# khanhptnk/magical-1

Measured on AMD Instinct MI355X. Metric: env-steps/sec (whole node) at N instances/GPU, 1/2/4/8 MI355X, higher is better.
Workload: dtype f64

## Files before the change

### include/magical_sim.h

```cpp
#ifndef MAGICAL_SIM_H
#define MAGICAL_SIM_H
#include <stdint.h>

#ifdef __cplusplus
extern "C" {
#endif

typedef struct mg_sim mg_sim;

typedef struct {
    int32_t task;
    int32_t rand_flags;
    int32_t preproc;
    int32_t num_envs;
    int32_t device;
    int32_t max_episode_steps;
    uint32_t base_seed;
    int32_t auto_reset;
    const uint32_t *seeds;
    const void *library;
    int64_t library_size;
} mg_config;

typedef struct {
// ... 25 lines not shown
int mg_read_timing(mg_sim *sim, double *out);
int mg_set_episode_steps(mg_sim *sim, const int32_t *steps_dev, void *stream);
int mg_replay_lores(const uint8_t *frames, int32_t nframes, const int32_t *episode_start, int32_t preproc,
                    uint8_t *scratch, uint8_t *out_allo, uint8_t *out_ego, uint8_t *out_past, void *stream);
int mg_restack(const uint8_t *recv, int32_t world, int32_t n, int64_t rank_stride, int64_t off_allo, int64_t off_ego,
               int64_t off_done, int32_t preproc, int64_t step, int32_t all_fresh, uint8_t *ring, uint8_t *out_allo,
               uint8_t *out_ego, uint8_t *out_past, void *stream);
int mg_restack_window(const uint8_t *recv, int32_t world, int32_t n, int64_t rank_stride, int64_t off_allo,
                      int64_t off_ego, int64_t off_done, int32_t preproc, int64_t step, int32_t all_fresh, int32_t K,
                      uint8_t *ring, void *stream);
int mg_bind_window(mg_sim *sim, uint8_t *ring_allo, uint8_t *ring_ego, int32_t K);
int mg_window_start(const mg_sim *sim, int32_t *slot);
int64_t mg_snapshot_bytes(const mg_config *cfg, int32_t n);
int mg_snapshot(mg_sim *sim, const int32_t *envs, int32_t n, uint8_t *blob_dev, void *stream);
int mg_restore(mg_sim *sim, const uint8_t *blob_dev, const int32_t *envs, const int32_t *recs, int32_t n, void *stream);
typedef struct {
    double  *score;
    int32_t *steps;
    double  *bodies;
    int32_t *counts;
    int32_t *errors;
} mg_lookahead_out;
int mg_lookahead(mg_sim *sim, const uint8_t *actions_dev, int32_t H, const mg_lookahead_out *out, void *stream);
#define MG_PLAN_MAX_ROLLOUTS 262144
typedef struct {
    int32_t *best;
    double  *best_score;
    uint8_t *first_action;
    double  *scores;
    int32_t *steps;
// ... 59 lines not shown
```

### magical-1_amd/csrc/mg_pool.h

```cpp
#pragma once
#include <hip/hip_runtime.h>
#include <functional>
#include <vector>
#include "mg_state.h"

enum { ROW_STATE = 0, ROW_RNG = 1 };
struct StateRow { uint64_t off; uint32_t esize, kind; };

__device__ __forceinline__ void copy_elem(char *dst, const char *src, uint32_t esize) {
    switch (esize) {
    case 8: *(uint64_t *)dst = *(const uint64_t *)src; break;
    case 4: *(uint32_t *)dst = *(const uint32_t *)src; break;
    case 2: *(uint16_t *)dst = *(const uint16_t *)src; break;
    default: *dst = *src; break;
    }
}

struct Carver {
    char *base;
    size_t off;
    std::vector<StateRow> *rows = nullptr;
    size_t N = 0;
    uint32_t kind = ROW_STATE;
    template <typename T> T *take(size_t n) {
        off = (off + 255) & ~(size_t)255;
        T *p = (T *)(base ? base + off : nullptr);
        if (rows)
            for (size_t k = 0; k < n / N; k++) rows->push_back(StateRow{off + k * N * sizeof(T), (uint32_t)sizeof(T), kind});
        off += n * sizeof(T);
        return p;
    }
};

inline void layout(MGState &S, Carver &c, bool frames = true) {
    size_t N = (size_t)S.N;
    c.N = N;
    size_t B = MG_MAX_BODIES * N, SH = MG_MAX_SHAPES * N, C = MG_MAX_CONS * N, A = MG_MAX_ARB * N, E = MG_MAX_ENTS * N;
    S.bpx = c.take<double>(B); S.bpy = c.take<double>(B); S.bvx = c.take<double>(B); S.bvy = c.take<double>(B);
    S.ba = c.take<double>(B); S.bw = c.take<double>(B); S.bvbx = c.take<double>(B); S.bvby = c.take<double>(B);
    S.bwb = c.take<double>(B); S.brc = c.take<double>(B); S.brs = c.take<double>(B); S.bminv = c.take<double>(B);
    S.biinv = c.take<double>(B); S.bacache = c.take<double>(B); S.bkin = c.take<int8_t>(B);
    S.nbodies = c.take<int32_t>(N);
    S.sbody = c.take<int8_t>(SH); S.spoly = c.take<int8_t>(SH); S.sent = c.take<int8_t>(SH);
    S.sgroup = c.take<int16_t>(SH); S.shash = c.take<int16_t>(SH); S.scat = c.take<uint8_t>(SH);
    S.sr = c.take<double>(SH); S.su = c.take<double>(SH); S.sbbl = c.take<double>(SH); S.sbbb = c.take<double>(SH);
    S.sbbr = c.take<double>(SH); S.sbbt = c.take<double>(SH);
    S.nshapes = c.take<int32_t>(N);
    S.ctype = c.take<int8_t>(C); S.ca = c.take<int8_t>(C); S.cb = c.take<int8_t>(C);
    S.cp = c.take<double>((size_t)CP_NUM * C);
// ... 13 lines not shown
    S.target_speed = c.take<double>(N); S.rel_turn = c.take<double>(N); S.target_finger = c.take<double>(N);
    S.robot_body0 = c.take<int32_t>(N); S.robot_cons0 = c.take<int32_t>(N); S.pv = c.take<double>(5 * N);
    S.ekind = c.take<int8_t>(E); S.etype = c.take<int8_t>(E); S.ecol = c.take<int8_t>(E); S.erole = c.take<int8_t>(E);
    S.ebody0 = c.take<int8_t>(E); S.eshape0 = c.take<int8_t>(E); S.enshapes = c.take<int8_t>(E);
    S.ex = c.take<double>(E); S.ey = c.take<double>(E); S.eang = c.take<double>(E); S.eh = c.take<double>(E);
    S.ew = c.take<double>(E); S.nents = c.take<int32_t>(N);
    S.goal_ent = c.take<int32_t>(N); S.episode_steps = c.take<int32_t>(N);
    S.tgt_ent = c.take<int32_t>(N); S.tgt_ids = c.take<int32_t>(2 * N);
    S.tgt_x = c.take<double>(N); S.tgt_y = c.take<double>(N);
    S.target_out = nullptr;
    c.kind = ROW_RNG;
    S.mt_key = c.take<uint32_t>(624 * N);
    c.kind = ROW_STATE;
    S.mt_pos = c.take<int32_t>(N);
    c.rows = nullptr;
    if (!frames) { S.hist_allo = S.hist_ego = S.scache = S.scache_ok = nullptr; S.hist_head = nullptr; return; }
    size_t FR = (size_t)MG_LORES * MG_LORES * 3;
    S.hist_allo = c.take<uint8_t>(4 * N * FR); S.hist_ego = c.take<uint8_t>(4 * N * FR);
    S.hist_head = c.take<int32_t>(2 * N);
    S.scache = c.take<uint8_t>(N * FR); S.scache_ok = c.take<uint8_t>(N);
}

struct StatePool { MGState S = {}; void *mem = nullptr; size_t bytes = 0; std::vector<StateRow> rows; };

inline void pool_free(StatePool &p) {
    (void)hipFree(p.mem);
    p = StatePool();
}

inline hipError_t pool_create(StatePool &p, const MGState &proto, int N, bool frames,
                              const std::function<void(Carver &)> &extra = nullptr) {
    p.S = proto;
    p.S.N = N;
    Carver sizing = {nullptr, 0};
    layout(p.S, sizing, frames);
    if (extra) extra(sizing);
    p.bytes = sizing.off + 256;
    hipError_t err = hipMalloc(&p.mem, p.bytes);
    if (err == hipSuccess) err = hipMemset(p.mem, 0, p.bytes);
    if (err != hipSuccess) { pool_free(p); return err; }
    Carver real = {(char *)p.mem, 0};
    real.rows = &p.rows;
    layout(p.S, real, frames);
    if (extra) extra(real);
    return hipSuccess;
// ... 10 lines not shown
```

### magical-1_amd/csrc/mg_render.h

```cpp
#pragma once
#include "mg_launch.h"
#include "mg_step.h"
#include "mg_prof.h"
#include <type_traits>

#define RG_LARGE 160, 1600, 256, 3072, 1600, MG_MAX_ENTS, uint32_t
#ifndef RG_MEDIUM0
#define RG_MEDIUM0 44, 784, 128, 1280, 512, MG_MAX_ENTS, uint16_t
#endif
#ifndef RG_MEDIUM1
#define RG_MEDIUM1 48, 896, 160, 1536, 512, MG_MAX_ENTS, uint16_t
#endif
#ifndef RG_MEDIUM2
#define RG_MEDIUM2 96, 1280, 160, 2560, 768, MG_MAX_ENTS, uint16_t, 16
#endif
#ifndef RG_SMALL
#define RG_SMALL 28, 640, 160, 1536, 208, 4, uint8_t, 16, 4
#endif
#define RG_MAXLONG 16
#define RG_MAXDE 16
#define RG_THREADS 192
#ifndef RG_SHORT
#define RG_SHORT 12
#endif
// ... 372 lines not shown
        } else if (x == MG_XF_PUPIL_L || x == MG_XF_PUPIL_R) {
            mg_transform_tr(0.0, 0.0, AT(S.ba, b + 2 + (x - MG_XF_PUPIL_L)) - AT(S.ba, b), xf);
        }
    } else if (kind == MG_ENT_BLOCK && x == MG_XF_MAIN) {
        const int b = AT(S.ebody0, ent);
        body_sincos(S, e, b, s, c);
        mg_transform_tr_sc(AT(S.bpx, b), AT(S.bpy, b), s, c, xf);
    } else if (kind == MG_ENT_GOAL && x == MG_XF_MAIN) {
        mg_transform_tr(AT(S.ex, ent), AT(S.ey, ent), 0.0, xf);
    }
}

template <class SM>
MG_DEV int xf_slot(int ent, int x) { return x == MG_XF_MAIN ? ent : SM::RG_MAXE + x - 1; }

#ifndef RG_SMALL_WPE
#define RG_SMALL_WPE 7
#endif
template <class SM, int MODE>
__global__ void __launch_bounds__(RG_THREADS)
__attribute__((amdgpu_waves_per_eu((SM::RG_MAXG <= 32 && RG_SMALL_WPE) ? RG_SMALL_WPE : 1)))
render_kernel(MGState S, const mg_library *__restrict__ L, RenderOut out) {
    __shared__ SM sm;
    constexpr int RG_BAND = SM::BAND, RG_NBANDS = SM::NBANDS, RG_BROWS = SM::BROWS;
    constexpr int RG_STKT = RG_BROWS * MG_LORES / 4, RG_RING0 = RG_STKT > 64 ? RG_STKT : 64;
    constexpr int RG_BANDLO = RG_BROWS * RG_LOROW, RG_BANDLO16 = SM::BANDLO16;
    constexpr int RG_CPF0 = RG_THREADS - RG_BANDLO16 < 128 ? RG_THREADS - RG_BANDLO16 : 128;
    constexpr int mode = MODE == 2 ? 0 : MODE;
    constexpr bool WIN = MODE == 2;
    const int e = blockIdx.x, view = blockIdx.y, tid = threadIdx.x, lane = tid & 63;
// ... 1 lines not shown
    if (out.retry_in) {
        const bool restart = out.cls_level == out.first_level && S.episode_steps[e] == 0;
        const int stored = S.rg_retry[2 * e + view];
        const int lvl = restart || stored < out.first_level ? out.first_level : stored;
        if (lvl != out.cls_level) return;
        if (tid == 0 && stored != lvl) S.rg_retry[2 * e + view] = (uint8_t)lvl;
    }
    if (mode == 0 && view == 0 && tid == 0 && S.scache_ok && S.episode_steps[e] == 0) S.scache_ok[e] = 0;
    MG_PROF_BEGIN(tid == 0);
#define RG_FAIL() do { \
        if (tid == 0) { if (out.retry_out) S.rg_retry[2 * e + view] = (uint8_t)(out.cls_level + 1); \
                        else S.overflow[e] |= 4 << view; } \
        return; } while (0)
    const int nents = S.nents[e];
    if (nents > SM::RG_MAXE || (out.retry_out && out.force_retry > out.cls_level - out.first_level)) RG_FAIL();
    int my_r0 = 0, my_nr = 0;
    if (tid < nents) {
        int kind = AT(S.ekind, tid);
        if (kind == MG_ENT_ARENA) { my_r0 = L->arena_rpoly0; my_nr = L->arena_nrpoly; }
        else if (kind == MG_ENT_GOAL) { my_r0 = L->goal_rpoly0; my_nr = L->goal_nrpoly; }
        else if (kind == MG_ENT_ROBOT) { my_r0 = L->robot_rpoly0; my_nr = L->robot_nrpoly; }
        else { int t = AT(S.etype, tid); my_r0 = L->block_rpoly0[t]; my_nr = L->block_nrpoly[t]; }
        sm.u.pre.e_g0[tid + 1] = (int16_t)my_nr;
        sm.u.pre.e_r0[tid] = (int16_t)my_r0;
        sm.u.pre.ocnt[tid] = 0;
    }
    if (tid == 0) {
        sm.err = 0; sm.ndash = 0; sm.nsedge = 0; sm.nlong = 0; sm.u.pre.ndedge = 0; sm.u.pre.nconv = 0;
        sm.col[0] = pack_rgb(L->background);
        sm.u.pre.e_g0[0] = 0;
// ... 78 lines not shown
            const int gk = goff[k];
#else
            const int gk = sm.u.pre.e_g0[k];
#endif
            if (k < nents && gk <= g) { ent = k; g0 = gk; }
        }
        const int r = sm.u.pre.e_r0[ent] + g - g0;
        const mg_rpoly &rp = L->rpoly[r];
        const int ecol = AT(S.ecol, ent);
        sm.u.pre.g_rpoly[g] = (int16_t)r;
        sm.g_ent[g] = (int8_t)ent;
        if (rp.outline) {
            if (atomicAdd(&sm.u.pre.ocnt[ent], 1) != 0) sm.err = 6;
            sm.oord1[ent + 1] = (uint16_t)((2 * g + 2) << RG_OSH);
        }
        sm.g_nv[g] = (int16_t)rp.npts;
        sm.col[2 * g + 1] = ref_colour(L, rp.col_ref, ecol);
        sm.col[2 * g + 2] = rp.outline ? ref_colour(L, rp.ocol_ref, ecol) : 0ull;
    }
    RG_SYNC();
    if (tid < 64) wave_exclusive_scan(sm.g_nv, sm.g_voff, G, lane);
    MG_PROF(11);
    for (int g = tid; g < G; g += RG_THREADS) {
        const mg_rpoly &rp = L->rpoly[sm.u.pre.g_rpoly[g]];
        int ent = sm.g_ent[g];
        double M[9];
        for (int i = 0; i < 9; i++) M[i] = sm.u.pre.view[i];
        for (int k = rp.nxf - 1; k >= 0; k--) {
            int x = rp.xf[k];
            const double *T = x >= MG_XF_STATIC0 ? L->static_xf[x - MG_XF_STATIC0] : sm.u.pre.e_xf[xf_slot<SM>(ent, x)];
            mg_mat3_mul(M, T, M);
        }
        for (int i = 0; i < 6; i++) sm.u.pre.g_m[g][i] = M[i];
    }
    RG_SYNC();
    const int NV = sm.g_voff[G];
    if (NV > SM::RG_MAXVERT) RG_FAIL();
    for (int g = tid; g < G; g += RG_THREADS)
        for (int i = 0, v0 = sm.g_voff[g]; i < sm.g_nv[g]; i++) sm.v_geom[v0 + i] = (uint8_t)g;
    RG_SYNC();
// ... 164 lines not shown
    uint8_t *ring = view == 0 ? S.hist_allo : S.hist_ego;
    const size_t FR = (size_t)MG_LORES * MG_LORES * 3;
    const bool fresh = S.episode_steps[e] == 0;
    const int head = S.hist_head[view * S.N + e];
    const int nh = fresh ? 0 : ((head + 1) & 3);
    const int pp = out.preproc;
    const bool fo = out.frames_only != 0;
    const bool stacked0 = !fo && (pp == MG_PREPROC_LORESSTACK || (pp == MG_PREPROC_LORES4E && view == 1) ||
                                  (pp == MG_PREPROC_LORES4A && view == 0));
    uint8_t *const wring = (WIN && stacked0) ? out.wring[view] : nullptr;
    const bool win = WIN && wring != nullptr;
    const bool stacked = stacked0 && !win;
    const bool plain = fo || pp != MG_PREPROC_LORESSTACK;
    const bool keep_ring = stacked || (!fo && pp == MG_PREPROC_LORES3EA && view == 1);
    constexpr bool kLayer = RG_SCACHE && SM::RG_MAXG <= 32;
    const bool cview = kLayer && mode == 0 && view == 0 && out.scache_mode != 1 && !keep_ring && !stacked0 && plain;
    const bool mk_cache = cview && fresh && !SM::ORDMAX;
    const bool use_cache = cview && !fresh && S.scache_ok[e] != 0;
    uint8_t *const scache = S.scache + (size_t)e * FR;
    uint4 cpf = make_uint4(0, 0, 0, 0);
    uint8_t *o_plain = view == 0 ? out.obs_allo : out.obs_ego;
    uint8_t *o_stack = pp == MG_PREPROC_LORESSTACK ? o_plain : out.obs_past;
    const int oyl = lane >> 5, ox = 32 * (tid >> 6) + (lane & 31), x0 = 4 * ox;
    const bool do_pf = mode == 0 && stacked && !fresh && tid < RG_STKT;
#ifdef MG_PROFILE
    const int dskip = out.debug_skip;
#else
    const int dskip = 0;
#endif
    uint32_t pf[3][3];
    auto prefetch = [&](int y0) {
#pragma unroll
        for (int k = 0; k < 3; k++) {
            const int sl = (nh + 1 + k) & 3;
// ... 234 lines not shown
                    uint32_t w0, w1;
                    if constexpr (SM::MPW == 8) { w0 = sm.u.post.band[yb + r][ox >> 1] >> (16 * (ox & 1)); w1 = 0u; }
                    else if constexpr (SM::MPW == 4) { w0 = sm.u.post.band[yb + r][ox]; w1 = 0u; }
                    else { const uint2 t = *(const uint2 *)&sm.u.post.band[yb + r][2 * ox]; w0 = t.x; w1 = t.y; }
                    if (w0 | w1) {
#pragma unroll
                        for (int c = 0; c < 4; c++) {
                            const uint32_t wc = (SM::MPW >= 4 || c < 2) ? w0 : w1;
                            const uint32_t m = (wc >> (SM::MBITS * (c % SM::MPW))) & (sonly ? sm.smask : SM::MMASK);
                            const uint32_t oo = sm.oord1[m ? 32 - __clz((int)m) : 0];
                            o[r][c] = o[r][c] > oo ? o[r][c] : oo;
                        }
                    }
                }
            }
            uint64_t sum = 0;
#pragma unroll
            for (int r = 0; r < 4; r++)
#pragma unroll
                for (int c = 0; c < 4; c++) sum += *(const uint64_t *)((const char *)sm.col + (o[r][c] << (3 - RG_OSH)));
            if (mode == 1) {
                for (int r = 0; r < 4; r++) {
                    uint8_t *dst = out.full + ((((size_t)e * 2 + view) * MG_RES + y0 + yb + r) * MG_RES + x0) * 3;
                    for (int c = 0; c < 4; c++) {
                        const uint64_t cc = *(const uint64_t *)((const char *)sm.col + (o[r][c] << (3 - RG_OSH)));
                        dst[3 * c] = (uint8_t)cc; dst[3 * c + 1] = (uint8_t)(cc >> 16); dst[3 * c + 2] = (uint8_t)(cc >> 32);
                    }
                }
            } else {
                uint8_t *dst8 = sonly ? (uint8_t *)sm.u.post.los : lo8;
// ... 75 lines not shown
                dst[0] = make_uint4(o[0], o[1], o[2], o[3]);
                dst[1] = make_uint4(o[4], o[5], o[6], o[7]);
                dst[2] = make_uint4(o[8], o[9], o[10], o[11]);
            }
        }
        if (band_i + 1 < band1) {
            if (tid >= 128) band_list(y0 + RG_BAND);
            if (do_pf) prefetch(y0 + RG_BAND);
            cache_prefetch(y0 + RG_BAND);
        }
        RG_SYNC();
        MG_PROF(4);
    }
    if (sm.err) { if (tid == 0) S.overflow[e] |= 4 << view; }
    if (mode == 0 && tid == 0) S.hist_head[view * S.N + e] = nh;
    if (cview && fresh && tid == 0) S.scache_ok[e] = mk_cache ? 1 : 0;
    MG_PROF_END(16 * view);
}
#undef RG_FAIL
```

### magical-1_amd/csrc/mg_sim.hip

```cpp
#include <cstdio>
#include <cstring>
#include <cstdlib>

#include "mg_sim.h"
#include "mg_phys.h"
#include "mg_philox.h"

static thread_local std::string g_err;
int set_err(int code, const std::string &msg) {
    g_err = msg;
    return code;
}

__global__ void __launch_bounds__(64) bodies_kernel(MGState S, double *out, int32_t *counts) {
    int e = blockIdx.x * blockDim.x + threadIdx.x;
    if (e >= S.n_envs) return;
    for (int b = 0; b < MG_MAX_BODIES; b++) {
        double *o = out + ((size_t)e * MG_MAX_BODIES + b) * 6;
        if (b < S.nbodies[e]) {
            o[0] = AT(S.bpx, b); o[1] = AT(S.bpy, b); o[2] = AT(S.ba, b);
            o[3] = AT(S.bvx, b); o[4] = AT(S.bvy, b); o[5] = AT(S.bw, b);
        } else {
            for (int k = 0; k < 6; k++) o[k] = 0.0;
        }
// ... 145 lines not shown
    s->max_steps = cfg->max_episode_steps; s->auto_reset = cfg->auto_reset;
    auto env_int = [](const char *name, int unset) { const char *v = getenv(name); return v ? atoi(v) : unset; };
    MGState proto = {};
    proto.n_envs = cfg->num_envs;
    proto.cons_cap = MG_MAX_CONS;
    proto.arb_cap = MG_MAX_ARB;
    proto.max_tries = 10000;
    if (env_int("MG_DEBUG_MAX_TRIES", 0) > 0) proto.max_tries = env_int("MG_DEBUG_MAX_TRIES", 0);
    s->reset_waves = env_int("MG_RESET_WAVES", 0);
    s->no_fused_reset = env_int("MG_FUSED_RESET", 1) == 0;
    s->reset_waves_shadow = env_int("MG_RESET_WAVES_SHADOW", 256);
    s->copy_wg = env_int("MG_COPY_WG", 2048);
    s->force_render_retry = env_int("MG_DEBUG_RENDER_RETRY", 0);
    s->scache_mode = env_int("MG_DEBUG_SCACHE", 0);
    const int N = (cfg->num_envs + 63) / 64 * 64;
    hipError_t err = pool_create(s->main, proto, N, true);
    if (err != hipSuccess) return set_err(-12, std::string("mg_create: state pool: ") + hipGetErrorString(err));
    if (hipMalloc((void **)&s->dlib, sizeof(mg_library)) != hipSuccess) return set_err(-12, "mg_create: hipMalloc library");
    HIPC(hipMemcpy(s->dlib, cfg->library, sizeof(mg_library), hipMemcpyHostToDevice));
    s->caps = step_caps(cfg->task, cfg->rand_flags, ((const mg_library *)cfg->library)->block_nshapes[MG_SHAPE_STAR]);
    s->step_form = step_pick_form(s->caps, env_int("MG_STEP_VARIANT", -1));
    int cus = 256;
    (void)hipDeviceGetAttribute(&cus, hipDeviceAttributeMultiprocessorCount, s->device);
    s->step_blk = step_pick_blk(s->step_form, cfg->num_envs, cus, env_int("MG_STEP_BLK", 0), env_int("MG_STEP_BLK0", 0));
    if (hipMalloc((void **)&s->reset_mask, (size_t)N) != hipSuccess) return set_err(-12, "mg_create: hipMalloc mask");
    HIPC(hipMemset(s->reset_mask, 0, (size_t)N));
    bool prefetch = s->auto_reset && s->task != MG_TASK_MOVE_TO_REGION && s->task != MG_TASK_MOVE_TO_CORNER;
    if (const char *pf = getenv("MG_RESET_PREFETCH")) prefetch = s->auto_reset && atoi(pf) != 0;
    if (prefetch) {
        HIPC(pool_create(s->shadow, proto, N, false));
        const std::vector<StateRow> &rows = s->main.rows;
// ... 299 lines not shown
```

### magical-1_amd/csrc/mg_snapshot.h

```cpp
#pragma once
#include <hip/hip_runtime.h>
#include <stdint.h>
#include "mg_common.h"

#define MG_SNAP_MAGIC 0x4E53474Du
#define MG_SNAP_VERSION 1
#define MG_SNAP_HEADER_BYTES 256
#define MG_SNAP_FRAME_BYTES (MG_LORES * MG_LORES * 3)
#define MG_SNAP_MAX_FRAMES 8

struct SnapHeader {
    uint32_t magic, version;
    int32_t task, rand_flags, preproc;
    int32_t max_bodies, max_shapes, max_cons, max_arb, max_ents;
    int32_t nrows, nframes;
    int64_t state_bytes, record_bytes, count, total_bytes;
    uint8_t zero[MG_SNAP_HEADER_BYTES - 12 * 4 - 4 * 8];
};
static_assert(sizeof(SnapHeader) == MG_SNAP_HEADER_BYTES, "SnapHeader is the blob's first 256 bytes");

struct SnapRow { uint64_t off; uint32_t esize, pre; };

struct SnapFrames { int n; uint8_t *base[MG_SNAP_MAX_FRAMES]; };

static inline int snap_frame_count(int preproc) {
    switch (preproc) {
    case MG_PREPROC_LORES4E: case MG_PREPROC_LORES3EA: return 6;
    case MG_PREPROC_LORESSTACK: return 8;
    case MG_PREPROC_LORES4A: return 5;
    default: return 0;
    }
}

hipError_t mg_launch_snap_header(const SnapHeader &h, uint8_t *blob, hipStream_t st);
hipError_t mg_launch_snap_state(char *pool, char *state, const SnapRow *rows, int nrows, const int32_t *envs,
                                const int32_t *recs, int n, int64_t count, int to_blob, hipStream_t st);
hipError_t mg_launch_snap_frames(const SnapFrames &F, uint8_t *frames, const int32_t *envs, const int32_t *recs, int n,
                                 int to_blob, hipStream_t st);
struct SnapRebuild { const uint8_t *ring[2]; const int32_t *head[2]; uint8_t *plain[2]; uint8_t *stack[2]; int N; };
hipError_t mg_launch_snap_rebuild(const SnapRebuild &R, const int32_t *envs, int n, hipStream_t st);
hipError_t mg_launch_snap_target(const int32_t *tgt_ids, const double *tgt_x, const double *tgt_y, int N,
                                 double *target_out, const int32_t *envs, int n, hipStream_t st);
```

### magical-1_amd/csrc/mg_snapshot.hip

```cpp
#include <cstring>

#include "mg_sim.h"

#define SNAP_MAX_WG 2048
#define SNAP_ROWS_PER_WG 8

__global__ void __launch_bounds__(64) snap_header_kernel(SnapHeader h, uint32_t *blob) {
    blob[threadIdx.x] = ((const uint32_t *)&h)[threadIdx.x];
}

template <bool TO_BLOB>
__global__ void __launch_bounds__(256) snap_state_kernel(char *__restrict__ pool, char *__restrict__ state,
                                                         const SnapRow *__restrict__ rows, int nrows,
                                                         const int32_t *__restrict__ envs, const int32_t *__restrict__ recs,
                                                         int n, int64_t count) {
    const int nrb = (n + 255) / 256, nrg = (nrows + SNAP_ROWS_PER_WG - 1) / SNAP_ROWS_PER_WG;
    for (int64_t item = blockIdx.x; item < (int64_t)nrb * nrg; item += gridDim.x) {
        const int k = (int)(item % nrb) * 256 + threadIdx.x;
        if (k >= n) continue;
        const size_t e = envs ? envs[k] : k, rec = recs ? recs[k] : k;
        const int r0 = (int)(item / nrb) * SNAP_ROWS_PER_WG, r1 = r0 + SNAP_ROWS_PER_WG < nrows ? r0 + SNAP_ROWS_PER_WG : nrows;
        for (int r = r0; r < r1; r++) {
            const SnapRow w = rows[r];
            char *p = pool + w.off + e * w.esize;
// ... 59 lines not shown
            dst[2] = make_uint4(o[8], o[9], o[10], o[11]);
        }
    }
}

__global__ void __launch_bounds__(64) snap_target_kernel(const int32_t *__restrict__ tgt_ids, const double *__restrict__ tgt_x,
                                                         const double *__restrict__ tgt_y, int N, double *__restrict__ out,
                                                         const int32_t *__restrict__ envs, int n) {
    const int k = blockIdx.x * 64 + threadIdx.x;
    if (k >= n) return;
    const size_t e = envs ? envs[k] : k;
    double *t = out + 4 * e;
    t[0] = tgt_ids[e]; t[1] = tgt_ids[N + e]; t[2] = tgt_x[e]; t[3] = tgt_y[e];
}

static unsigned capped(int64_t items) { return (unsigned)(items < SNAP_MAX_WG ? (items > 0 ? items : 1) : SNAP_MAX_WG); }

hipError_t mg_launch_snap_header(const SnapHeader &h, uint8_t *blob, hipStream_t st) {
    hipLaunchKernelGGL(snap_header_kernel, dim3(1), dim3(64), 0, st, h, (uint32_t *)blob);
    return hipGetLastError();
}

hipError_t mg_launch_snap_state(char *pool, char *state, const SnapRow *rows, int nrows, const int32_t *envs,
                                const int32_t *recs, int n, int64_t count, int to_blob, hipStream_t st) {
    if (n <= 0 || nrows <= 0) return hipSuccess;
    const int64_t items = (int64_t)((n + 255) / 256) * ((nrows + SNAP_ROWS_PER_WG - 1) / SNAP_ROWS_PER_WG);
    if (to_blob)
        hipLaunchKernelGGL(snap_state_kernel<true>, dim3(capped(items)), dim3(256), 0, st, pool, state, rows, nrows, envs,
                           recs, n, count);
    else
        hipLaunchKernelGGL(snap_state_kernel<false>, dim3(capped(items)), dim3(256), 0, st, pool, state, rows, nrows, envs,
                           recs, n, count);
    return hipGetLastError();
}

hipError_t mg_launch_snap_frames(const SnapFrames &F, uint8_t *frames, const int32_t *envs, const int32_t *recs, int n,
                                 int to_blob, hipStream_t st) {
    if (n <= 0 || F.n <= 0) return hipSuccess;
    const int64_t items = (int64_t)n * F.n;
    if (to_blob)
        hipLaunchKernelGGL(snap_frames_kernel<true>, dim3(capped(items)), dim3(192), 0, st, F, frames, envs, recs, n);
    else
        hipLaunchKernelGGL(snap_frames_kernel<false>, dim3(capped(items)), dim3(192), 0, st, F, frames, envs, recs, n);
    return hipGetLastError();
}

hipError_t mg_launch_snap_rebuild(const SnapRebuild &R, const int32_t *envs, int n, hipStream_t st) {
    if (n <= 0 || (!R.ring[0] && !R.ring[1])) return hipSuccess;
    const int64_t blocks = ((int64_t)n * (MG_LORES * MG_LORES / 4) + 255) / 256;
    hipLaunchKernelGGL(snap_rebuild_kernel, dim3(capped(blocks), 2), dim3(256), 0, st, R, envs, n);
    return hipGetLastError();
}

hipError_t mg_launch_snap_target(const int32_t *tgt_ids, const double *tgt_x, const double *tgt_y, int N,
                                 double *target_out, const int32_t *envs, int n, hipStream_t st) {
    if (n <= 0) return hipSuccess;
    hipLaunchKernelGGL(snap_target_kernel, dim3((n + 63) / 64), dim3(64), 0, st, tgt_ids, tgt_x, tgt_y, N, target_out,
                       envs, n);
// ... 99 lines not shown
        HIPC(hipEventCreateWithFlags(&s->ev_snap, hipEventDisableTiming));
    }
    if (s->snap_inflight) HIPC(hipEventSynchronize(s->ev_snap));
    s->snap_inflight = 0;
    int32_t *he = (int32_t *)s->snap_stage, *hr = he + ne;
    uint8_t *hm = (uint8_t *)(hr + ne);
    for (int k = 0; k < n; k++) { he[k] = envs ? envs[k] : k; hr[k] = recs ? recs[k] : k; }
    if (want_mask) {
        memset(hm, 0, (size_t)s->main.S.N);
        for (int k = 0; k < n; k++) hm[he[k]] = 1;
    }
    HIPC(hipMemcpyAsync(s->snap_dev, s->snap_stage, bytes, hipMemcpyHostToDevice, st));
    *envs_dev = (const int32_t *)s->snap_dev;
    *recs_dev = *envs_dev + ne;
    if (mask_dev) *mask_dev = (const uint8_t *)(*recs_dev + ne);
    return 0;
}

int mg_snapshot(mg_sim *s, const int32_t *envs, int32_t n, uint8_t *blob, void *stream) {
    if (!s || !blob) return set_err(-22, "mg_snapshot: null argument");
    if ((uintptr_t)blob & 15) return set_err(-22, "mg_snapshot: the blob must be 16-byte aligned");
    if (int rc = snap_check_mode(s, "mg_snapshot")) return rc;
    if (n <= 0 || n > s->main.S.n_envs || (!envs && n != s->main.S.n_envs))
        return set_err(-22, "mg_snapshot: n must be in [1, num_envs], and num_envs when envs is null");
    for (int k = 0; envs && k < n; k++)
        if (envs[k] < 0 || envs[k] >= s->main.S.n_envs) return set_err(-22, "mg_snapshot: env index out of range");
    HIPC(hipSetDevice(s->device));
    hipStream_t st = as_stream(stream);
    const int32_t *de = nullptr, *dr = nullptr;
    if (envs) {
// ... 45 lines not shown
        const int64_t r = recs ? recs[k] : k;
        if (r < 0 || r >= h.count) return set_err(-22, "mg_restore: record index out of range (the blob holds " +
                                                            std::to_string(h.count) + ")");
    }
    const bool all = n == ne;
    const int32_t *de = nullptr, *dr = nullptr;
    const uint8_t *dm = nullptr;
    const bool staged = envs || recs || !all;
    if (staged) {
        if (int rc = snap_stage_indices(s, st, envs, recs, n, true, &de, &dr, &dm)) return rc;
        if (all) dm = nullptr;
    }
    const char *state = (const char *)blob + MG_SNAP_HEADER_BYTES;
    HIPC(mg_launch_snap_state((char *)s->main.mem, (char *)state, s->srows, s->nsrows, de, dr, n, h.count, 0, st));
    HIPC(mg_launch_snap_frames(snap_frames(s), (uint8_t *)state + h.count * h.state_bytes, de, dr, n, 0, st));
    SnapRebuild R;
    memset(&R, 0, sizeof(R));
    R.N = s->main.S.N;
    const int pp = s->preproc;
    if (pp == MG_PREPROC_LORESSTACK || pp == MG_PREPROC_LORES4A) {
        R.ring[0] = s->main.S.hist_allo; R.head[0] = s->main.S.hist_head;
        R.plain[0] = pp == MG_PREPROC_LORES4A ? s->out.obs_allo : nullptr;
        R.stack[0] = pp == MG_PREPROC_LORES4A ? s->out.obs_past : s->out.obs_allo;
    }
    if (pp == MG_PREPROC_LORESSTACK || pp == MG_PREPROC_LORES4E || pp == MG_PREPROC_LORES3EA) {
        R.ring[1] = s->main.S.hist_ego; R.head[1] = s->main.S.hist_head + s->main.S.N;
        R.plain[1] = pp == MG_PREPROC_LORESSTACK ? nullptr : s->out.obs_ego;
        R.stack[1] = pp == MG_PREPROC_LORESSTACK ? s->out.obs_ego : pp == MG_PREPROC_LORES4E ? s->out.obs_past : nullptr;
    }
    HIPC(mg_launch_snap_rebuild(R, de, n, st));
// ... 14 lines not shown
```

### magical-1_amd/csrc/mg_state.h

```cpp
#pragma once
#include "mg_common.h"

struct MGState {
    int N;
    int n_envs;
    int cons_cap, arb_cap;
    int max_tries;
    double *bpx, *bpy, *bvx, *bvy, *ba, *bw, *bvbx, *bvby, *bwb, *brc, *brs, *bminv, *biinv, *bacache;
    int8_t *bkin;
    int32_t *nbodies;
    int8_t *sbody, *spoly, *sent;
    int16_t *sgroup, *shash;
    uint8_t *scat;
    double *sr, *su, *sbbl, *sbbb, *sbbr, *sbbt;
    int32_t *nshapes;
    int8_t *ctype, *ca, *cb;
    double *cp;
    int32_t *ncons;
    int32_t *akey;
    uint32_t *astamp;
    int8_t *astate, *acount, *asa, *asb;
    double *anx, *any, *au;
    double *acon;
    uint64_t *ahash;
// ... 10 lines not shown
    double *ex, *ey, *eang, *eh, *ew;
    int32_t *nents;
    int32_t *goal_ent;
    int32_t *episode_steps;
    int32_t *tgt_ent, *tgt_ids;
    double *tgt_x, *tgt_y;
    double *target_out;
    uint32_t *mt_key;
    int32_t *mt_pos;
    uint32_t *mt_lds;
    uint8_t *hist_allo;
    uint8_t *hist_ego;
    int32_t *hist_head;
    uint8_t *scache;
    uint8_t *scache_ok;
};

enum {
    CP_MAXF = 0, CP_MAXB = 1, CP_BCOEF = 2, CP_JACC = 3, CP_JACC2 = 4, CP_ISUM = 5, CP_BIAS = 6, CP_BIAS2 = 7,
    CP_AAX = 8, CP_AAY = 9, CP_ABX = 10, CP_ABY = 11, CP_R1X = 12, CP_R1Y = 13, CP_R2X = 14, CP_R2Y = 15,
    CP_K11 = 16, CP_K12 = 17, CP_K21 = 18, CP_K22 = 19,
    CP_PHASE = 8, CP_RATIO = 9, CP_RATIO_INV = 10,
    CP_MIN = 8, CP_MAX = 9,
    CP_RATE = 8,
    CP_REST = 8, CP_STIFF = 9, CP_WCOEF = 10, CP_TWRN = 11,
    CP_NUM = 20
};
enum { AC_R1X = 0, AC_R1Y, AC_R2X, AC_R2Y, AC_NMASS, AC_TMASS, AC_JN, AC_JT, AC_JB, AC_BIAS, AC_NUM };
enum { ARB_FIRST = 0, ARB_NORMAL = 1, ARB_CACHED = 3 };
```

### magical-1_amd/magical_amd/envs.py

```python
import collections
import ctypes

import numpy as np
import torch

from . import native, registry, spaces, tables
from .planning import as_objective

_LIBRARY = None


def library():
    global _LIBRARY
    if _LIBRARY is None:
        _LIBRARY = tables.build_library()
    return _LIBRARY


def _obs_shapes(spec):
    pp = spec.preproc
    if pp is None:
        return collections.OrderedDict([("allo", (384, 384, 3)), ("ego", (384, 384, 3))])
    if pp == "LoResStack":
        return collections.OrderedDict([("allo", (96, 96, 12)), ("ego", (96, 96, 12))])
# ... 233 lines not shown
        out = (ctypes.c_int32 * 6)()
        native.check(self.lib.mg_step_form(self.handle, out))
        return int(out[0]), int(out[1]), tuple(int(x) for x in out[2:6])

    def arbiters(self):
        out = torch.empty((self.num_envs, 48, 28), dtype=torch.float64, device=self.device)
        hs = torch.empty((self.num_envs, 48, 2), dtype=torch.uint64, device=self.device)
        native.check(self.lib.mg_get_arbiters(self.handle, ctypes.c_void_p(out.data_ptr()),
                                              ctypes.c_void_p(hs.data_ptr()), self._stream()))
        return out, hs

    def set_body_pose(self, env, body, x, y, angle):
        native.check(self.lib.mg_set_body_pose(self.handle, int(env), int(body), float(x), float(y), float(angle),
                                               self._stream()))

    def errors(self):
        out = torch.empty(self.num_envs, dtype=torch.int32, device=self.device)
        native.check(self.lib.mg_get_errors(self.handle, ctypes.c_void_p(out.data_ptr()), self._stream()))
        return out

    def snapshot_bytes(self, n=None):
        nbytes = self.lib.mg_snapshot_bytes(ctypes.byref(self._cfg), self.num_envs if n is None else int(n))
        if nbytes < 0:
            native.check(int(nbytes))
        return int(nbytes)

    def snapshot(self, envs=None, out=None):
        from .snapshot import Snapshot
        n = self.num_envs if envs is None else len(envs)
        nbytes = self.snapshot_bytes(n)
# ... 330 lines not shown
```

### magical-1_amd/magical_amd/native.py

```python
import ctypes
import os

HERE = os.path.dirname(os.path.abspath(__file__))
LIB_PATH = os.path.join(HERE, "libmagical_sim_prof.so" if os.environ.get("MAGICAL_AMD_PROFILE") == "1"
                        else "libmagical_sim.so")
if os.environ.get("MAGICAL_AMD_EXP_LIB"):
    LIB_PATH = os.path.join(HERE, "libmagical_sim_%s.so" % os.path.basename(os.environ["MAGICAL_AMD_EXP_LIB"]))

EXPORTS = ["mg_create", "mg_bind_outputs", "mg_reset", "mg_step", "mg_render_full", "mg_get_bodies", "mg_get_arbiters",
           "mg_set_body_pose", "mg_get_errors", "mg_seed", "mg_random_actions", "mg_num_envs", "mg_step_form", "mg_enable_timing", "mg_read_timing",
           "mg_set_episode_steps", "mg_selftest_sincos", "mg_replay_lores", "mg_restack", "mg_restack_window", "mg_bind_window",
           "mg_window_start", "mg_snapshot_bytes", "mg_snapshot", "mg_restore", "mg_lookahead", "mg_plan", "mg_plan_sample",
           "mg_plan_cem", "mg_lookahead_obj", "mg_plan_obj", "mg_plan_cem_obj", "mg_plan_beam", "mg_destroy", "mg_last_error"]
PLAN_MAX_ROLLOUTS = 262144
OBJ_FINAL, OBJ_RETURN, OBJ_PEAK = 0, 1, 2


class mg_config(ctypes.Structure):
    _fields_ = [("task", ctypes.c_int32), ("rand_flags", ctypes.c_int32), ("preproc", ctypes.c_int32),
                ("num_envs", ctypes.c_int32), ("device", ctypes.c_int32), ("max_episode_steps", ctypes.c_int32),
                ("base_seed", ctypes.c_uint32), ("auto_reset", ctypes.c_int32),
                ("seeds", ctypes.POINTER(ctypes.c_uint32)), ("library", ctypes.c_void_p),
                ("library_size", ctypes.c_int64)]


class mg_buffers(ctypes.Structure):
    _fields_ = [("obs_allo", ctypes.c_void_p), ("obs_ego", ctypes.c_void_p), ("obs_past", ctypes.c_void_p),
# ... 77 lines not shown
    if hasattr(lib, "mg_replay_lores"):
        lib.mg_replay_lores.argtypes = [vp, i32, vp, i32, vp, vp, vp, vp, vp]
    if hasattr(lib, "mg_restack"):
        i64 = ctypes.c_int64
        lib.mg_restack.argtypes = [vp, i32, i32, i64, i64, i64, i64, i32, i64, i32, vp, vp, vp, vp, vp]
    if hasattr(lib, "mg_restack_window"):
        i64 = ctypes.c_int64
        lib.mg_restack_window.argtypes = [vp, i32, i32, i64, i64, i64, i64, i32, i64, i32, i32, vp, vp]
    if hasattr(lib, "mg_bind_window"):
        lib.mg_bind_window.argtypes = [vp, vp, vp, i32]
        lib.mg_window_start.argtypes = [vp, ctypes.POINTER(i32)]
    lib.mg_snapshot_bytes.argtypes = [ctypes.POINTER(mg_config), i32]
    lib.mg_snapshot_bytes.restype = ctypes.c_int64
    lib.mg_snapshot.argtypes = [vp, ctypes.POINTER(i32), i32, vp, vp]
    lib.mg_restore.argtypes = [vp, vp, ctypes.POINTER(i32), ctypes.POINTER(i32), i32, vp]
    lib.mg_lookahead.argtypes = [vp, vp, i32, ctypes.POINTER(mg_lookahead_out), vp]
    lib.mg_plan.argtypes = [vp, vp, i32, i32, ctypes.POINTER(mg_plan_out), vp]
    lib.mg_plan_sample.argtypes = [vp, vp, i32, i32, i32, u64, u64, vp]
    lib.mg_plan_cem.argtypes = [vp, vp, vp, i32, i32, i32, i32, i32, i32, i32, u64, u64,
                                ctypes.POINTER(mg_plan_cem_out), vp]
    po = ctypes.POINTER(mg_objective)
    lib.mg_lookahead_obj.argtypes = [vp, vp, i32, po, ctypes.POINTER(mg_lookahead_out), ctypes.POINTER(mg_objective_out), vp]
    lib.mg_plan_obj.argtypes = [vp, vp, i32, i32, po, ctypes.POINTER(mg_plan_out), vp]
    lib.mg_plan_cem_obj.argtypes = [vp, vp, vp, i32, i32, i32, i32, i32, i32, i32, u64, u64, po,
                                    ctypes.POINTER(mg_plan_cem_out), vp]
    lib.mg_plan_beam.argtypes = [vp, vp, vp, i32, i32, i32, i32, po, ctypes.POINTER(mg_plan_beam_out), vp]
    lib.mg_destroy.argtypes = [vp]
    lib.mg_destroy.restype = None
    lib.mg_last_error.restype = ctypes.c_char_p
    for name in EXPORTS[:-2]:
# ... 14 lines not shown
```

Measured before the change: 3.477 million.

## Cache static-layer ordering per env to render only dynamic bodies

```diff
diff --git a/include/magical_sim.h b/include/magical_sim.h
--- a/include/magical_sim.h
+++ b/include/magical_sim.h
@@ -63,6 +63,8 @@
 int64_t mg_snapshot_bytes(const mg_config *cfg, int32_t n);
 int mg_snapshot(mg_sim *sim, const int32_t *envs, int32_t n, uint8_t *blob_dev, void *stream);
 int mg_restore(mg_sim *sim, const uint8_t *blob_dev, const int32_t *envs, const int32_t *recs, int32_t n, void *stream);
+int mg_layer_levels(mg_sim *sim, uint8_t *out_host);
+int32_t mg_restored_layer_level(int32_t stored);
 typedef struct {
     double  *score;
     int32_t *steps;
diff --git a/magical-1_amd/csrc/mg_pool.h b/magical-1_amd/csrc/mg_pool.h
--- a/magical-1_amd/csrc/mg_pool.h
+++ b/magical-1_amd/csrc/mg_pool.h
@@ -32,7 +32,8 @@
     }
 };
 
-inline void layout(MGState &S, Carver &c, bool frames = true) {
+enum { FRAMES_NONE = 0, FRAMES = 1, FRAMES_SORD = 2 };
+inline void layout(MGState &S, Carver &c, int frames = FRAMES) {
     size_t N = (size_t)S.N;
     c.N = N;
     size_t B = MG_MAX_BODIES * N, SH = MG_MAX_SHAPES * N, C = MG_MAX_CONS * N, A = MG_MAX_ARB * N, E = MG_MAX_ENTS * N;
@@ -76,11 +77,18 @@
     c.kind = ROW_STATE;
     S.mt_pos = c.take<int32_t>(N);
     c.rows = nullptr;
+    S.sord = nullptr;
     if (!frames) { S.hist_allo = S.hist_ego = S.scache = S.scache_ok = nullptr; S.hist_head = nullptr; return; }
     size_t FR = (size_t)MG_LORES * MG_LORES * 3;
     S.hist_allo = c.take<uint8_t>(4 * N * FR); S.hist_ego = c.take<uint8_t>(4 * N * FR);
     S.hist_head = c.take<int32_t>(2 * N);
     S.scache = c.take<uint8_t>(N * FR); S.scache_ok = c.take<uint8_t>(N);
+    if (frames == FRAMES_SORD) S.sord = c.take<uint8_t>(N * (size_t)MG_LORES * MG_LORES * 16);
+}
+
+inline bool sord_applies(int task, int preproc) {
+    return (task == MG_TASK_MOVE_TO_REGION || task == MG_TASK_MOVE_TO_CORNER) &&
+           (preproc == MG_PREPROC_LORES4E || preproc == MG_PREPROC_LORES3EA);
 }
 
 struct StatePool { MGState S = {}; void *mem = nullptr; size_t bytes = 0; std::vector<StateRow> rows; };
@@ -90,7 +98,7 @@
     p = StatePool();
 }
 
-inline hipError_t pool_create(StatePool &p, const MGState &proto, int N, bool frames,
+inline hipError_t pool_create(StatePool &p, const MGState &proto, int N, int frames,
                               const std::function<void(Carver &)> &extra = nullptr) {
     p.S = proto;
     p.S.N = N;
diff --git a/magical-1_amd/csrc/mg_render.h b/magical-1_amd/csrc/mg_render.h
--- a/magical-1_amd/csrc/mg_render.h
+++ b/magical-1_amd/csrc/mg_render.h
@@ -410,6 +410,12 @@
 template <class SM>
 MG_DEV int xf_slot(int ent, int x) { return x == MG_XF_MAIN ? ent : SM::RG_MAXE + x - 1; }
 
+MG_DEV bool layer_view(const RenderOut &out, int view) {
+    const int pp = out.preproc;
+    return view == 0 && out.scache_mode != 1 &&
+           (out.frames_only != 0 || (pp != MG_PREPROC_LORESSTACK && pp != MG_PREPROC_LORES4A));
+}
+
 #ifndef RG_SMALL_WPE
 #define RG_SMALL_WPE 7
 #endif
@@ -441,6 +447,11 @@
         return; } while (0)
     const int nents = S.nents[e];
     if (nents > SM::RG_MAXE || (out.retry_out && out.force_retry > out.cls_level - out.first_level)) RG_FAIL();
+    constexpr bool kOrd = RG_SCACHE && SM::RG_MAXG <= 32 && !SM::ORDMAX && MODE == 0;
+    bool body_only = false;
+    if constexpr (kOrd)
+        body_only = layer_view(out, view) && out.scache_mode != 3 && S.sord != nullptr && S.episode_steps[e] != 0 &&
+                    S.scache_ok[e] == 2;
     int my_r0 = 0, my_nr = 0;
     if (tid < nents) {
         int kind = AT(S.ekind, tid);
@@ -549,7 +560,8 @@
             if (atomicAdd(&sm.u.pre.ocnt[ent], 1) != 0) sm.err = 6;
             sm.oord1[ent + 1] = (uint16_t)((2 * g + 2) << RG_OSH);
         }
-        sm.g_nv[g] = (int16_t)rp.npts;
+        if constexpr (kOrd) sm.g_nv[g] = (int16_t)((body_only && ((sm.smask >> ent) & 1u)) ? 0 : rp.npts);
+        else sm.g_nv[g] = (int16_t)rp.npts;
         sm.col[2 * g + 1] = ref_colour(L, rp.col_ref, ecol);
         sm.col[2 * g + 2] = rp.outline ? ref_colour(L, rp.ocol_ref, ecol) : 0ull;
     }
@@ -559,6 +571,8 @@
     for (int g = tid; g < G; g += RG_THREADS) {
         const mg_rpoly &rp = L->rpoly[sm.u.pre.g_rpoly[g]];
         int ent = sm.g_ent[g];
+        if constexpr (kOrd)
+            if (body_only && ((sm.smask >> ent) & 1u)) continue;
         double M[9];
         for (int i = 0; i < 9; i++) M[i] = sm.u.pre.view[i];
         for (int k = rp.nxf - 1; k >= 0; k--) {
@@ -753,10 +767,12 @@
     const bool plain = fo || pp != MG_PREPROC_LORESSTACK;
     const bool keep_ring = stacked || (!fo && pp == MG_PREPROC_LORES3EA && view == 1);
     constexpr bool kLayer = RG_SCACHE && SM::RG_MAXG <= 32;
-    const bool cview = kLayer && mode == 0 && view == 0 && out.scache_mode != 1 && !keep_ring && !stacked0 && plain;
+    const bool cview = kLayer && mode == 0 && layer_view(out, view);
     const bool mk_cache = cview && fresh && !SM::ORDMAX;
     const bool use_cache = cview && !fresh && S.scache_ok[e] != 0;
     uint8_t *const scache = S.scache + (size_t)e * FR;
+    const bool mk_ord = kOrd && mk_cache && out.scache_mode != 3 && S.sord != nullptr;
+    uint4 *const sord = kOrd ? (uint4 *)S.sord + (size_t)e * (MG_LORES * MG_LORES) : nullptr;
     uint4 cpf = make_uint4(0, 0, 0, 0);
     uint8_t *o_plain = view == 0 ? out.obs_allo : out.obs_ego;
     uint8_t *o_stack = pp == MG_PREPROC_LORESSTACK ? o_plain : out.obs_past;
@@ -1021,6 +1037,30 @@
                     }
                 }
             }
+            if constexpr (kOrd && !sonly) {
+                if (body_only && out.scache_mode != 4) {
+                    const uint4 so4 = sord[(y0 / 4 + oy) * MG_LORES + ox];
+#pragma unroll
+                    for (int r = 0; r < 4; r++) {
+                        const uint32_t sw = r == 0 ? so4.x : r == 1 ? so4.y : r == 2 ? so4.z : so4.w;
+#pragma unroll
+                        for (int c = 0; c < 4; c++) {
+                            const uint32_t s = ((sw >> (8 * c)) & 0xFFu) << RG_OSH;
+                            o[r][c] = o[r][c] > s ? o[r][c] : s;
+                        }
+                    }
+                }
+            }
+            if constexpr (kOrd && sonly) {
+                if (mk_ord) {
+                    uint32_t w[4];
+#pragma unroll
+                    for (int r = 0; r < 4; r++)
+                        w[r] = (o[r][0] >> RG_OSH) | ((o[r][1] >> RG_OSH) << 8) | ((o[r][2] >> RG_OSH) << 16) |
+                               ((o[r][3] >> RG_OSH) << 24);
+                    sord[(y0 / 4 + oy) * MG_LORES + ox] = make_uint4(w[0], w[1], w[2], w[3]);
+                }
+            }
             uint64_t sum = 0;
 #pragma unroll
             for (int r = 0; r < 4; r++)
@@ -1126,7 +1166,7 @@
     }
     if (sm.err) { if (tid == 0) S.overflow[e] |= 4 << view; }
     if (mode == 0 && tid == 0) S.hist_head[view * S.N + e] = nh;
-    if (cview && fresh && tid == 0) S.scache_ok[e] = mk_cache ? 1 : 0;
+    if (cview && fresh && tid == 0) S.scache_ok[e] = mk_cache ? (mk_ord ? 2 : 1) : 0;
     MG_PROF_END(16 * view);
 }
 #undef RG_FAIL
diff --git a/magical-1_amd/csrc/mg_sim.hip b/magical-1_amd/csrc/mg_sim.hip
--- a/magical-1_amd/csrc/mg_sim.hip
+++ b/magical-1_amd/csrc/mg_sim.hip
@@ -183,7 +183,7 @@
     s->force_render_retry = env_int("MG_DEBUG_RENDER_RETRY", 0);
     s->scache_mode = env_int("MG_DEBUG_SCACHE", 0);
     const int N = (cfg->num_envs + 63) / 64 * 64;
-    hipError_t err = pool_create(s->main, proto, N, true);
+    hipError_t err = pool_create(s->main, proto, N, sord_applies(cfg->task, cfg->preproc) ? FRAMES_SORD : FRAMES);
     if (err != hipSuccess) return set_err(-12, std::string("mg_create: state pool: ") + hipGetErrorString(err));
     if (hipMalloc((void **)&s->dlib, sizeof(mg_library)) != hipSuccess) return set_err(-12, "mg_create: hipMalloc library");
     HIPC(hipMemcpy(s->dlib, cfg->library, sizeof(mg_library), hipMemcpyHostToDevice));
diff --git a/magical-1_amd/csrc/mg_snapshot.h b/magical-1_amd/csrc/mg_snapshot.h
--- a/magical-1_amd/csrc/mg_snapshot.h
+++ b/magical-1_amd/csrc/mg_snapshot.h
@@ -32,6 +32,9 @@
     }
 }
 
+__host__ __device__ static inline uint8_t snap_restored_scache_ok(uint8_t stored) { return stored > 1 ? 1 : stored; }
+hipError_t mg_launch_snap_demote(uint8_t *scache_ok, const int32_t *envs, int n, hipStream_t st);
+
 hipError_t mg_launch_snap_header(const SnapHeader &h, uint8_t *blob, hipStream_t st);
 hipError_t mg_launch_snap_state(char *pool, char *state, const SnapRow *rows, int nrows, const int32_t *envs,
                                 const int32_t *recs, int n, int64_t count, int to_blob, hipStream_t st);
diff --git a/magical-1_amd/csrc/mg_snapshot.hip b/magical-1_amd/csrc/mg_snapshot.hip
--- a/magical-1_amd/csrc/mg_snapshot.hip
+++ b/magical-1_amd/csrc/mg_snapshot.hip
@@ -97,6 +97,14 @@
     t[0] = tgt_ids[e]; t[1] = tgt_ids[N + e]; t[2] = tgt_x[e]; t[3] = tgt_y[e];
 }
 
+__global__ void __launch_bounds__(256) snap_demote_kernel(uint8_t *__restrict__ scache_ok, const int32_t *__restrict__ envs,
+                                                          int n) {
+    for (int k = blockIdx.x * 256 + threadIdx.x; k < n; k += gridDim.x * 256) {
+        const size_t e = envs ? envs[k] : k;
+        scache_ok[e] = snap_restored_scache_ok(scache_ok[e]);
+    }
+}
+
 static unsigned capped(int64_t items) { return (unsigned)(items < SNAP_MAX_WG ? (items > 0 ? items : 1) : SNAP_MAX_WG); }
 
 hipError_t mg_launch_snap_header(const SnapHeader &h, uint8_t *blob, hipStream_t st) {
@@ -125,6 +133,12 @@
         hipLaunchKernelGGL(snap_frames_kernel<true>, dim3(capped(items)), dim3(192), 0, st, F, frames, envs, recs, n);
     else
         hipLaunchKernelGGL(snap_frames_kernel<false>, dim3(capped(items)), dim3(192), 0, st, F, frames, envs, recs, n);
+    return hipGetLastError();
+}
+
+hipError_t mg_launch_snap_demote(uint8_t *scache_ok, const int32_t *envs, int n, hipStream_t st) {
+    if (n <= 0 || !scache_ok) return hipSuccess;
+    hipLaunchKernelGGL(snap_demote_kernel, dim3(capped((n + 255) / 256)), dim3(256), 0, st, scache_ok, envs, n);
     return hipGetLastError();
 }
 
@@ -254,6 +268,19 @@
     *envs_dev = (const int32_t *)s->snap_dev;
     *recs_dev = *envs_dev + ne;
     if (mask_dev) *mask_dev = (const uint8_t *)(*recs_dev + ne);
+    return 0;
+}
+
+int32_t mg_restored_layer_level(int32_t stored) {
+    return snap_restored_scache_ok((uint8_t)(stored < 0 ? 0 : stored > 255 ? 255 : stored));
+}
+
+int mg_layer_levels(mg_sim *s, uint8_t *out_host) {
+    if (!s || !out_host) return set_err(-22, "mg_layer_levels: null argument");
+    HIPC(hipSetDevice(s->device));
+    HIPC(hipDeviceSynchronize());
+    if (!s->main.S.scache_ok) { memset(out_host, 0, (size_t)s->main.S.n_envs); return 0; }
+    HIPC(hipMemcpy(out_host, s->main.S.scache_ok, (size_t)s->main.S.n_envs, hipMemcpyDeviceToHost));
     return 0;
 }
 
@@ -329,6 +356,7 @@
     const char *state = (const char *)blob + MG_SNAP_HEADER_BYTES;
     HIPC(mg_launch_snap_state((char *)s->main.mem, (char *)state, s->srows, s->nsrows, de, dr, n, h.count, 0, st));
     HIPC(mg_launch_snap_frames(snap_frames(s), (uint8_t *)state + h.count * h.state_bytes, de, dr, n, 0, st));
+    HIPC(mg_launch_snap_demote(s->main.S.scache_ok, de, n, st));
     SnapRebuild R;
     memset(&R, 0, sizeof(R));
     R.N = s->main.S.N;
diff --git a/magical-1_amd/csrc/mg_state.h b/magical-1_amd/csrc/mg_state.h
--- a/magical-1_amd/csrc/mg_state.h
+++ b/magical-1_amd/csrc/mg_state.h
@@ -48,6 +48,7 @@
     int32_t *hist_head;
     uint8_t *scache;
     uint8_t *scache_ok;
+    uint8_t *sord;
 };
 
 enum {
diff --git a/magical-1_amd/magical_amd/envs.py b/magical-1_amd/magical_amd/envs.py
--- a/magical-1_amd/magical_amd/envs.py
+++ b/magical-1_amd/magical_amd/envs.py
@@ -271,6 +271,11 @@
         native.check(self.lib.mg_set_body_pose(self.handle, int(env), int(body), float(x), float(y), float(angle),
                                                self._stream()))
 
+    def layer_levels(self):
+        out = (ctypes.c_uint8 * self.num_envs)()
+        native.check(self.lib.mg_layer_levels(self.handle, out))
+        return list(out)
+
     def errors(self):
         out = torch.empty(self.num_envs, dtype=torch.int32, device=self.device)
         native.check(self.lib.mg_get_errors(self.handle, ctypes.c_void_p(out.data_ptr()), self._stream()))
diff --git a/magical-1_amd/magical_amd/native.py b/magical-1_amd/magical_amd/native.py
--- a/magical-1_amd/magical_amd/native.py
+++ b/magical-1_amd/magical_amd/native.py
@@ -10,7 +10,7 @@
 EXPORTS = ["mg_create", "mg_bind_outputs", "mg_reset", "mg_step", "mg_render_full", "mg_get_bodies", "mg_get_arbiters",
            "mg_set_body_pose", "mg_get_errors", "mg_seed", "mg_random_actions", "mg_num_envs", "mg_step_form", "mg_enable_timing", "mg_read_timing",
            "mg_set_episode_steps", "mg_selftest_sincos", "mg_replay_lores", "mg_restack", "mg_restack_window", "mg_bind_window",
-           "mg_window_start", "mg_snapshot_bytes", "mg_snapshot", "mg_restore", "mg_lookahead", "mg_plan", "mg_plan_sample",
+           "mg_window_start", "mg_snapshot_bytes", "mg_snapshot", "mg_restore", "mg_layer_levels", "mg_restored_layer_level", "mg_lookahead", "mg_plan", "mg_plan_sample",
            "mg_plan_cem", "mg_lookahead_obj", "mg_plan_obj", "mg_plan_cem_obj", "mg_plan_beam", "mg_destroy", "mg_last_error"]
 PLAN_MAX_ROLLOUTS = 262144
 OBJ_FINAL, OBJ_RETURN, OBJ_PEAK = 0, 1, 2
@@ -118,6 +118,9 @@
     lib.mg_snapshot_bytes.restype = ctypes.c_int64
     lib.mg_snapshot.argtypes = [vp, ctypes.POINTER(i32), i32, vp, vp]
     lib.mg_restore.argtypes = [vp, vp, ctypes.POINTER(i32), ctypes.POINTER(i32), i32, vp]
+    if hasattr(lib, "mg_layer_levels"):
+        lib.mg_layer_levels.argtypes = [vp, vp]
+        lib.mg_restored_layer_level.argtypes = [i32]
     lib.mg_lookahead.argtypes = [vp, vp, i32, ctypes.POINTER(mg_lookahead_out), vp]
     lib.mg_plan.argtypes = [vp, vp, i32, i32, ctypes.POINTER(mg_plan_out), vp]
     lib.mg_plan_sample.argtypes = [vp, vp, i32, i32, i32, u64, u64, vp]
```

New measurement: 3.361 million. -3.3%, worse.
